# zhouzypaul/fql

Hardware: AMD Instinct MI355X
Metric: FQL gradient-steps/s (batch=256) (higher is better)
Workload: dtype f32

## Files before the change

fql_amd/csrc/fql_engine.hip:

```cpp
#include "../../include/fql_amd.h"
#include "fql_kernels.h"
#include "fql_conv.h"
#include "fql_chain.h"
#include "fql_aux.h"
#include "fql_ifql.h"
#include "fql_rebrac.h"
#include "fql_sac.h"
#include "fql_bc.h"
#include "fql_iql.h"
#include "fql_iqld.h"
#include "fql_cfgrl.h"
#include <hip/hip_ext.h>
#include "fql_aql.h"

#include <algorithm>
#include <cmath>
#include <cstdarg>
#include <cstdio>
#include <cstdlib>
#include <cstring>
#include <map>
#include <memory>
#include <random>
#include <string>
// ... 108 lines not shown
    size_t off = 0;
    ((off = ((off + alignof(T) - 1) & ~(alignof(T) - 1)) + sizeof(T)), ...);
    return off;
}
template <typename... Pm, typename... A>
Bound bind(void (*k)(Pm...), int grid, A&&... a) {
    static_assert(sizeof...(Pm) == sizeof...(A) && sizeof...(Pm) <= 2, "a bound launch takes the kernel's one or two arguments");
    static_assert(packed_bytes<Pm...>() <= FQL_BOUND_BYTES, "argument struct larger than Bound::args: raise FQL_BOUND_BYTES");
    Bound b;
    b.fn = (const void*)k;
    b.grid = (unsigned)grid;
    size_t off = 0;
    int n = 0;
    auto put = [&](auto v) {
        using T = decltype(v);
        off = (off + alignof(T) - 1) & ~(alignof(T) - 1);
        b.at[n++] = (int)off;
        std::memcpy(b.args + off, &v, sizeof(T));
        off += sizeof(T);
    };
    (put(static_cast<Pm>(a)), ...);
    b.len = (int)off;
    return b;
}

struct Op {
    OpType type;
    std::vector<const void*> reads, writes;
    GemmTask gemm;
    WgradTask wgrad;
    LnBwdTask ln;
    PrepArgs prep;
    PostOsArgs postos;
    LossCriticArgs lc;
    LossQArgs lq;
    LossBcArgs lb;
    LossActorArgs la;
    EulerFinishArgs ef;
    ConvArgs conv;
    PoolArgs pool;
    PoolBwdArgs poolb;
    ConvWgradArgs cw;
    ConvWredArgs cwr;
    EncDzArgs edz;
    ChainArgs chain;
    const ConvWprepTask* wprep_tasks = nullptr;
    int wprep_n = 0;
    int cw_grid = 0;
    int adam_c0 = 0, adam_n = -1;
    int adam_c1 = 0, adam_n1 = 0;
    int adam_polyak = -1;
    float adam_lr = 0.f;
    DevState* adam_st = nullptr;
    int fin_mode = 0;
    Bound k;
    int level = 0;
    int lane = 0;
    std::vector<int> deps;
};

struct Launch {
    OpType type;
    int grid = 0, ntasks = 0;
    size_t lds = 0;
    void* table = nullptr;
    Op op;
    bool pool_fused = false;
    int lane = 0;
    bool tmt2 = false, kbig = false, euler = false;
    double macs = 0.0;
    void *table_w = nullptr, *table_l = nullptr, *table_m = nullptr;
    int n_w = 0, n_l = 0, tile_w = 0, tile_l = 0, tile_m = 0;
    std::vector<GemmTask> dg_tasks;
    std::vector<GemmTask> h_gemm;
    std::vector<WgradTask> h_wgrad;
    std::vector<LnBwdTask> h_ln;
    std::vector<MiscTask> h_misc;
    std::shared_ptr<const SideArgs> ka_side;
    std::vector<int> waits;
    bool record_after = false;
    hipEvent_t ev = nullptr;
};

inline bool ka_tasks_env() {
    const char* e = getenv("FQL_KERNARG_TASKS");
    return !e || atoi(e) != 0;
}
inline std::shared_ptr<const SideArgs> ka_side_args(const Launch& L) {
    const size_t ng = L.h_gemm.size(), nw = L.h_wgrad.size(), nl = L.h_ln.size(), nm = L.h_misc.size();
    if (ng > FQL_KA_GEMM || nw > FQL_KA_WGRAD || nl > FQL_KA_LN || nm > FQL_KA_MISC) return nullptr;
    auto a = std::make_shared<SideArgs>();
    std::memset(a.get(), 0, sizeof(SideArgs));
    SideFront& f = a->f;
    f.tile_w = L.tile_w; f.tile_l = L.tile_l; f.tile_m = L.tile_m; f.tl = -1;
    for (int& v : f.g0) v = FQL_KA_FRONT_PAD;
    for (int& v : f.w0) v = FQL_KA_FRONT_PAD;
    for (int& v : f.l0) v = FQL_KA_FRONT_PAD;
    for (size_t i = 0; i < ng; ++i) { a->g[i] = L.h_gemm[i]; if (i) f.g0[i - 1] = L.h_gemm[i].tile0; }
    for (size_t i = 0; i < nw; ++i) { a->w[i] = L.h_wgrad[i]; if (i) f.w0[i - 1] = L.h_wgrad[i].tile0; }
    for (size_t i = 0; i < nl; ++i) { a->l[i] = L.h_ln[i]; if (i) f.l0[i - 1] = L.h_ln[i].tile0; }
    for (size_t i = 0; i < nm; ++i) a->m[i] = L.h_misc[i];
    return a;
}
struct Program {
    std::vector<Op> ops;
    std::vector<Launch> launches;
    bool lane_used[FQL_LANES] = {};
    hipEvent_t ev_fork = nullptr, ev_join[FQL_LANES] = {};
    hipGraph_t graph = nullptr;
    hipGraphExec_t exec = nullptr;
    int64_t macs = 0;
    AqlProgram aql;
    bool aql_tried = false;
};

template <typename P, typename IssueFn>
void issue_lanes(P& pr, hipStream_t s0, const hipStream_t* ls, bool fork, IssueFn&& issue) {
    auto lazy = [](hipEvent_t& e) { if (!e) HIP_CHECK(hipEventCreateWithFlags(&e, hipEventDisableTiming)); };
    bool side = false;
    if (ls) for (int l = 1; l < FQL_LANES; ++l) side |= pr.lane_used[l];
    if (side && fork) {
        lazy(pr.ev_fork);
        HIP_CHECK(hipEventRecord(pr.ev_fork, s0));
        for (int l = 1; l < FQL_LANES; ++l) if (pr.lane_used[l]) HIP_CHECK(hipStreamWaitEvent(ls[l], pr.ev_fork, 0));
    }
    for (auto& L : pr.launches) {
        const hipStream_t s = side && L.lane != 0 ? ls[L.lane] : s0;
        if (side)
            for (int w : L.waits) if (pr.launches[w].ev) HIP_CHECK(hipStreamWaitEvent(s, pr.launches[w].ev, 0));
        issue(L, s);
        if (side && L.record_after) {
            lazy(L.ev);
            HIP_CHECK(hipEventRecord(L.ev, s));
        }
    }
    if (side)
        for (int l = 1; l < FQL_LANES; ++l) {
            if (!pr.lane_used[l]) continue;
// ... 170 lines not shown
    int64_t* cf_rows = nullptr;
    uint32_t* cf_draws = nullptr;
    bool own_info() const { return kind == AgentKind::IQL || kind == AgentKind::IQLD; }
    uint64_t seed = 0;
    int device = 0;
    hipStream_t stream = nullptr;
    hipStream_t lane_streams[FQL_LANES] = {};
    bool allow64 = true;
    int emit_lane = 0;
    std::vector<Op>* defer_wgrads = nullptr;
    std::string err;

    Net nets[NUM_NETS];
    EncNet encs[NUM_ENC];
    ConvWprepTask* enc_wprep[NUM_ENC] = {nullptr, nullptr, nullptr, nullptr};
    int enc_nconv[NUM_ENC] = {0, 0, 0, 0};
    std::vector<void*> enc_allocs;
    bool visual = false;
    int enc_dim = 0;
    unsigned char* img_all = nullptr;
    EncBuf eb_c, eb_t, eb_bc, eb_os;
    size_t n_train = 0, n_total = 0, critic_size = 0;
    float *P = nullptr, *G = nullptr, *Mu = nullptr, *Nu = nullptr;
    std::vector<Leaf> leaves;
    int n_train_leaves = 0;
    AdamChunk* d_chunks = nullptr;
    float* d_partials = nullptr;
    int* d_leaf_range = nullptr;
    int n_chunks = 0;

    DevState* d_state = nullptr;
    SrcDesc* d_src = nullptr;
    SrcDesc h_src_shadow{};
    bool src_valid = false;
    SrcDesc* h_src_ring = nullptr;
    int src_ring_pos = 0;

    int B = 0;
    std::vector<void*> ws_allocs;
    float *in_obs = nullptr, *in_act = nullptr, *in_rew = nullptr, *in_mask = nullptr, *in_nobs = nullptr, *in_nact = nullptr;
    float* in_noise[5] = {nullptr, nullptr, nullptr, nullptr, nullptr};
    int64_t* in_idx = nullptr;
    float *X_os = nullptr, *X_bc = nullptr, *X_eu = nullptr, *X_c1 = nullptr, *X_c2 = nullptr, *X_ct = nullptr;
    float *vel = nullptr, *w_rew = nullptr, *w_mask = nullptr, *w_act = nullptr, *tgt = nullptr;
    float *X_e0 = nullptr, *C0 = nullptr, *Abuf[2] = {nullptr, nullptr}, *Vpart = nullptr;
    bool fused_euler = false;
    bool use_chain = false;
    int fill_lane_full = 1;
    std::vector<float*> wf_bc;
    float *wf_w0 = nullptr, *wf_w4 = nullptr;
    WfragTask* d_wfrag = nullptr;
    int wfrag_n = 0, wfrag_grid = 0;
    const bool ka_tasks = ka_tasks_env();
    std::vector<void*> chain_allocs;
    bool split_build = false;
    bool wide_tiles = false;
    bool split_ok = false;
    int vp_tiles = 0;
    int num_cus = 0;
    PassBuf p_os, p_os_bwd, p_bc, p_eu, p_c1[2], p_c2[2], p_ct[2];
    Program prog_fwdbwd, prog_opt, prog_loss;
    Program prog_opt_split;
    Program prog_full;
    int mod_chunk0[3] = {0, 0, 0}, mod_chunkn[3] = {0, 0, 0};
    Program prog_split;
    hipGraphExec_t split_exec[4] = {nullptr, nullptr, nullptr, nullptr};
    hipGraph_t split_graph[4] = {nullptr, nullptr, nullptr, nullptr};
    hipEvent_t ev_a = nullptr, ev_b = nullptr, ev_c = nullptr;
    bool split_begun = false;
    bool began = false;
    AqlRuntime aql;
    std::vector<AqlDispatch>* aql_rec = nullptr;
    bool last_update_aql = false;
    bool hip_dirty = true;
    void aql_drain() {
        if (!aql.up) return;
        try { aql.drain(); } catch (const AqlError& e) { throw HipError{e.msg}; }
    }

    float *ds_obs = nullptr, *ds_act = nullptr, *ds_rew = nullptr, *ds_mask = nullptr, *ds_nobs = nullptr;
    float* ds_row = nullptr;
    int64_t ds_size = 0, ds_cap = 0, ds_ptr = 0;
    unsigned char *ds_frames = nullptr, *ds_next_frames = nullptr;
    int64_t* ds_init = nullptr;
    int ds_fs = 0;
    float ds_paug = 0.f;
    float *rb_obs = nullptr, *rb_act = nullptr, *rb_rew = nullptr, *rb_mask = nullptr, *rb_nobs = nullptr;
    unsigned char *rb_frames = nullptr, *rb_next_frames = nullptr;
    int64_t* rb_init = nullptr;
    int64_t rb_size = 0, rb_cap = 0, rb_ptr = 0;
    int64_t* in_init = nullptr;
    int *in_crop = nullptr, *in_crop_user = nullptr;

    struct Eval {
        int n_pad = 0;
        std::vector<void*> allocs;
        float *X = nullptr, *Xf = nullptr, *tgt = nullptr;
        PassBuf p_os, p_eu;
        Program prog_os, prog_flow;
        float *st_obs = nullptr, *st_noise = nullptr, *st_out = nullptr;
        float* st_goal = nullptr;
        float *Xf2 = nullptr, *cfgs = nullptr;
        unsigned char* st_img = nullptr;
        EncBuf eb_os, eb_bc;
        Program prog_enc_os, prog_enc_bc;
        float* Xq = nullptr;
// ... 354 lines not shown
            lf.name = "modules_unc_embed/Embed_0/embedding";
            lf.ndim = 2;
            lf.shape[0] = 1; lf.shape[1] = gcfg.goal_dim; lf.shape[2] = lf.shape[3] = 1;
            lf.segs.push_back(Segment{emb_off, 1, gcfg.goal_dim, 1, pad16(gcfg.goal_dim)});
            lf.trainable = true;
            lf.train_id = tid++;
            leaves.push_back(lf);
        }
        n_train_leaves = tid;
        if (n_train_leaves > 256) invalid("too many trainable leaves (%d)", n_train_leaves);
        std::vector<AdamChunk> ch;
        for (const Leaf& lf : leaves) {
            if (!lf.trainable) continue;
            for (const Segment& s : lf.segs) {
                if (s.chunk_w > 0) {
                    for (int r = 0; r < s.rows_p; ++r) ch.push_back(AdamChunk{(int)(s.off + (size_t)r * s.cols_p), s.chunk_w, lf.train_id});
                    continue;
                }
                const size_t len = (size_t)s.rows_p * s.cols_p;
                for (size_t o = 0; o < len; o += 4096)
                    ch.push_back(AdamChunk{(int)(s.off + o), (int)std::min<size_t>(4096, len - o), lf.train_id});
            }
        }
        n_chunks = (int)ch.size();
        HIP_CHECK(hipMalloc((void**)&d_chunks, ch.size() * sizeof(AdamChunk)));
        HIP_CHECK(hipMemcpy(d_chunks, ch.data(), ch.size() * sizeof(AdamChunk), hipMemcpyHostToDevice));
        std::vector<int> range(n_train_leaves + 1, 0);
        for (const AdamChunk& c : ch) range[c.leaf + 1]++;
        for (int i = 0; i < n_train_leaves; ++i) range[i + 1] += range[i];
        {
            static const char* const trained[kNumKinds][3] = {
                {"modules_actor_bc_flow/", "modules_actor_onestep_flow/", "modules_critic/"},
                {"modules_actor_flow/", "modules_value/", "modules_critic/"},
                {"modules_actor/", "modules_critic/", "modules_critic/"},
                {"modules_actor/", "modules_alpha/", "modules_critic/"},
                {nullptr, nullptr, nullptr},
                {"modules_actor/", "modules_value/", "modules_critic/"},
                {"actor/", "value/", "critic/"},
                {nullptr, nullptr, nullptr}};
            const char* const* mods = trained[(int)kind];
            for (int m = 0; m < 3; ++m) {
                if (!mods[m]) { mod_chunk0[m] = 0; mod_chunkn[m] = n_chunks; continue; }
                int lo = 1 << 30, hi = -1;
                for (const Leaf& lf : leaves)
                    if (lf.trainable && lf.name.rfind(mods[m], 0) == 0) { lo = std::min(lo, lf.train_id); hi = std::max(hi, lf.train_id); }
                mod_chunk0[m] = range[lo];
                mod_chunkn[m] = range[hi + 1] - range[lo];
            }
        }
        HIP_CHECK(hipMalloc((void**)&d_leaf_range, range.size() * sizeof(int)));
        HIP_CHECK(hipMemcpy(d_leaf_range, range.data(), range.size() * sizeof(int), hipMemcpyHostToDevice));
        HIP_CHECK(hipMalloc((void**)&d_partials, (size_t)n_chunks * 4 * sizeof(float)));
        HIP_CHECK(hipMemset(d_partials, 0, (size_t)n_chunks * 4 * sizeof(float)));
    }

    const Leaf* find_leaf(const char* name) const {
        for (const Leaf& l : leaves)
            if (l.name == name) return &l;
        return nullptr;
    }
    static size_t leaf_count(const Leaf& l) {
        size_t n = 1;
        for (int i = 0; i < l.ndim; ++i) n *= (size_t)l.shape[i];
        return n;
    }
    void leaf_io(const Leaf& lf, float* arena, float* host, bool to_device) {
        HIP_CHECK(hipStreamSynchronize(stream));
        size_t ho = 0;
        for (const Segment& s : lf.segs) {
            HIP_CHECK(hipMemcpy2D(to_device ? (void*)(arena + s.off) : (void*)(host + ho), (to_device ? s.cols_p : s.cols) * sizeof(float),
                                  to_device ? (const void*)(host + ho) : (const void*)(arena + s.off),
                                  (to_device ? s.cols : s.cols_p) * sizeof(float), s.cols * sizeof(float), s.rows,
                                  to_device ? hipMemcpyHostToDevice : hipMemcpyDeviceToHost));
            ho += (size_t)s.rows * s.cols;
        }
    }

    void init_params() {
        std::vector<float> h(n_total, 0.f);
        std::mt19937_64 gen(seed * 0x9E3779B97F4A7C15ull + 0x1234567ull);
        for (int ni = 0; ni <= NET_OS; ++ni)
            for (const Layer& L : nets[ni].layers) {
                const bool actor_head = ni == NET_BC && &L == &nets[ni].layers.back();
                const double scale = !actor_head ? 1.0 : kind == AgentKind::REBRAC ? (double)rcfg.actor_fc_scale
                                     : kind == AgentKind::IQL ? 1e-2
                                                              : 1.0;
                if ((kind == AgentKind::BC || kind == AgentKind::IQLD) && actor_head) {
                    const double sd = std::sqrt(1.0 / (double)L.in) / 0.87962566103423978;
                    std::normal_distribution<double> Nd(0.0, 1.0);
                    for (int r = 0; r < L.in; ++r)
                        for (int c = 0; c < L.out; ++c) {
                            double v = Nd(gen);
                            while (v < -2.0 || v > 2.0) v = Nd(gen);
                            h[L.w + (size_t)r * L.out_p + c] = (float)(sd * v);
                        }
                    continue;
                }
                if (kind == AgentKind::SAC && actor_head) {
                    const int ad = cfg.act_dim, ap = pad16(ad);
                    const double lim = std::sqrt(6.0 * (double)scfg.actor_fc_scale / (double)(L.in + ad));
                    std::uniform_real_distribution<double> U(-lim, lim);
                    for (int c0 : {0, ap})
                        for (int r = 0; r < L.in; ++r)
                            for (int c = 0; c < ad; ++c) h[L.w + (size_t)r * L.out_p + c0 + c] = (float)U(gen);
                    continue;
                }
// ... 1118 lines not shown
            case OP_POOL_BWD: {
                const PoolBwdArgs& a = L.op.poolb;
                const size_t tot = (size_t)a.N * a.H * a.W * (a.C / 4);
                FQL_LAUNCH(fql_maxpool_bwd_kernel, dim3((unsigned)((tot + FQL_THREADS - 1) / FQL_THREADS)), dim3(FQL_THREADS), 0, s, a);
                break;
            }
            case OP_CONV_WGRAD:
                if (cfg.precision == 2) FQL_LAUNCH(fql_conv_wgrad_split_kernel, dim3(L.grid), dim3(FQL_THREADS), L.lds, s, (const ConvWgradArgs*)L.table, L.ntasks);
                else
                FQL_LAUNCH(fql_conv_wgrad_kernel, dim3(L.grid), dim3(FQL_THREADS), L.lds, s, (const ConvWgradArgs*)L.table, L.ntasks);
                break;
            case OP_CONV_WRED:
                FQL_LAUNCH(fql_conv_wgrad_reduce_kernel, dim3(L.grid), dim3(FQL_THREADS), 0, s, (const ConvWredArgs*)L.table, L.ntasks);
                break;
            case OP_ENC_DZ: {
                const EncDzArgs& a = L.op.edz;
                FQL_LAUNCH(fql_enc_dz_kernel, dim3((a.M * a.n + FQL_THREADS - 1) / FQL_THREADS), dim3(FQL_THREADS), 0, s, a);
                break;
            }
            case OP_CHAIN: {
                ChainArgs ca = L.op.chain; ca.tl = tl;
                ca.xg = chain_xg(ca.M, cfg.actor_hidden[0]);
                if (cfg.precision == 2 && ca.variant != 3) {
#define FQL_CHAIN_SPLIT(HH, VV) FQL_LAUNCH((fql_chain_split_kernel<HH, VV>), dim3((L.op.chain.M / 16) * (HH / 32)), dim3(FQL_CHAIN_THREADS), FQL_CHAIN_LDS_BYTES(HH), s, ca)
                    if (cfg.actor_hidden[0] == 512) { if (ca.variant == 0) FQL_CHAIN_SPLIT(512, 0); else if (ca.variant == 1) FQL_CHAIN_SPLIT(512, 1); else FQL_CHAIN_SPLIT(512, 2); }
                    else { if (ca.variant == 0) FQL_CHAIN_SPLIT(256, 0); else if (ca.variant == 1) FQL_CHAIN_SPLIT(256, 1); else FQL_CHAIN_SPLIT(256, 2); }
#undef FQL_CHAIN_SPLIT
                }
                else {
#define FQL_CHAIN_F32(HH, VV) FQL_LAUNCH((fql_chain_kernel<HH, VV>), dim3((L.op.chain.M / 16) * (HH / 32)), dim3(FQL_CHAIN_THREADS), FQL_CHAIN_LDS_BYTES(HH), s, ca)
                    if (cfg.actor_hidden[0] == 512) { if (ca.variant == 0) FQL_CHAIN_F32(512, 0); else if (ca.variant == 1) FQL_CHAIN_F32(512, 1); else if (ca.variant == 2) FQL_CHAIN_F32(512, 2); else FQL_CHAIN_F32(512, 3); }
                    else { if (ca.variant == 0) FQL_CHAIN_F32(256, 0); else if (ca.variant == 1) FQL_CHAIN_F32(256, 1); else if (ca.variant == 2) FQL_CHAIN_F32(256, 2); else FQL_CHAIN_F32(256, 3); }
#undef FQL_CHAIN_F32
                }
                break;
            }
            case OP_WFRAG:
                FQL_LAUNCH(fql_wfrag_kernel, dim3(wfrag_grid), dim3(FQL_THREADS), 0, s, (const WfragTask*)d_wfrag, wfrag_n, tl);
                break;
            case OP_DGRAD0: {
                Dgrad0Args a{};
                a.ntasks = (int)L.dg_tasks.size(); a.col0 = L.op.gemm.i1;
                for (int i = 0; i < a.ntasks; ++i) a.t[i] = L.dg_tasks[i];
                FQL_LAUNCH(fql_dgrad0_kernel, dim3(a.ntasks * (L.op.gemm.M / 16)), dim3(FQL_THREADS), 0, s, a);
                break;
            }
            case OP_HEAD_DGRAD:
                FQL_LAUNCH(fql_head_dgrad_kernel, dim3((L.op.gemm.M / 16) * (L.op.gemm.N / 64)), dim3(FQL_THREADS), 0, s, L.op.gemm);
                break;
            case OP_ADAM: {
                AdamArgs a{P, G, Mu, Nu, P + n_train, d_chunks, L.op.adam_st ? L.op.adam_st : d_state, d_partials, L.op.adam_c0,
                           L.op.adam_polyak >= 0 ? L.op.adam_polyak : (int)critic_size, L.op.adam_lr > 0.f ? L.op.adam_lr : cfg.lr, cfg.tau, tl,
                           L.op.adam_n1 > 0 ? L.op.adam_n : -1, L.op.adam_c1};
                FQL_LAUNCH(fql_adam_kernel, dim3(L.op.adam_n < 0 ? n_chunks : L.op.adam_n + L.op.adam_n1), dim3(FQL_THREADS), 0, s, a);
                break;
            }
            case OP_FINALIZE:
                FQL_LAUNCH(fql_finalize_kernel, dim3(1), dim3(FQL_THREADS), 0, s,
                                   FinalizeArgs{d_state, d_chunks, d_partials, d_leaf_range, n_chunks, n_train_leaves, L.op.fin_mode, tl});
                break;
            case OP_WGRAD: case OP_LNBWD: case OP_POSTOS: case OP_LOSS_CRITIC: case OP_LOSS_Q: case OP_LOSS_BC:
            case OP_PEC: case OP_XCHAIN: case OP_NUM_TYPES:
                throw HipError{"internal: op type " + std::to_string((int)L.type) + " has no launch of its own"};
            default: {
                const Bound& k = L.op.k;
                if (!k.fn) throw HipError{"internal: op type " + std::to_string((int)L.type) + " carries no bound launch"};
                alignas(16) unsigned char a[FQL_BOUND_BYTES];
                std::memcpy(a, k.args, (size_t)k.len);
                if (k.tl_at >= 0) std::memcpy(a + k.tl_at, &tl, sizeof tl);
                if (L.type == OP_IQLD_CFG) std::memcpy(a + offsetof(IqldCfgStepArgs, cfg), &sample_cfg, sizeof sample_cfg);
                void* argv[2] = {a + k.at[0], a + k.at[1]};
                if (aql_rec) aql_rec->push_back(AqlDispatch{k.fn, {k.grid, 1, 1}, {FQL_THREADS, 1, 1}, 0, std::vector<uint8_t>(a, a + k.len)});
                else if (prof_a) (void)hipExtLaunchKernel(k.fn, dim3(k.grid), dim3(FQL_THREADS), argv, 0, s, prof_a, prof_b, 0);
                else (void)hipLaunchKernel(k.fn, dim3(k.grid), dim3(FQL_THREADS), argv, 0, s);
                break;
            }
        }
    }

#undef FQL_LAUNCH
    void issue_of(const Program& pr, const Launch& L, hipStream_t s) {
        issue(L, s, &pr == &prog_full ? (int)(&L - pr.launches.data()) : -1);
    }
    void run_launches(Program& pr, hipStream_t s0, const hipStream_t* ls = nullptr, bool fork = true) {
        static const bool trace_l = getenv("FQL_TRACE") != nullptr;
        issue_lanes(pr, s0, ls, fork, [&](const Launch& L, hipStream_t s) {
            if (trace_l) {
                fprintf(stderr, "[fql] launch %d type %d lane %d grid %d waits %zu:", (int)(&L - pr.launches.data()), (int)L.type, L.lane, L.grid, L.waits.size());
                for (int w : L.waits) fprintf(stderr, " %d(lane %d)", w, pr.launches[w].lane);
                fprintf(stderr, "\n");
            }
            issue_of(pr, L, s);
        });
    }
    std::vector<AqlDispatch> record_dispatches(const Program& pr) {
        std::vector<AqlDispatch> rec;
        aql_rec = &rec;
        try {
            for (const Launch& L : pr.launches) issue_of(pr, L, nullptr);
        } catch (...) { aql_rec = nullptr; throw; }
        aql_rec = nullptr;
        if (rec.size() != pr.launches.size()) throw HipError{"internal: a launch did not record exactly one dispatch"};
        return rec;
    }

    void build_aql(Program& pr) {
// ... 394 lines not shown
                        if (m == 2) a.writes.push_back(P + n_train + c.w);
                    }
                const Layer& D = encs[ei].dense;
                a.reads.push_back(G + D.w); a.reads.push_back(G + D.b);
                a.writes.push_back(P + D.w);
                if (m == 2) a.writes.push_back(P + n_train + D.w);
            }
            for (int ni : net_ids)
                for (const Layer& L : nets[ni].layers) {
                    a.reads.push_back(G + L.w); a.reads.push_back(G + L.b);
                    a.writes.push_back(P + L.w);
                    if (L.ln) { a.reads.push_back(G + L.g); a.reads.push_back(G + L.be); a.writes.push_back(P + L.g); }
                    if (ni == NET_C0 || ni == NET_C1) a.writes.push_back(P + n_train + L.w);
                }
            emit_lane = lane;
            push(pr, a);
        }

    void build_opt_program(Program& pr, bool two_lanes) {
        DevState* st = d_state;
        if (two_lanes) {
            adam_for(pr, 2, {NET_C0, NET_C1}, 1);
            adam_for(pr, 0, {NET_BC}, 1);
            if (use_chain) { emit_lane = 1; emit_wfrag(pr); }
            adam_for(pr, 1, {NET_OS}, 0);
        } else {
            adam_for(pr, 2, {NET_C0, NET_C1, NET_BC, NET_OS}, 0, -2);
            if (use_chain) { emit_lane = 0; emit_wfrag(pr); }
        }
        Op f{};
        f.type = OP_FINALIZE;
        f.fin_mode = 1;
        f.reads = {d_partials + mod_chunk0[0] * 4, d_partials + mod_chunk0[1] * 4, d_partials + mod_chunk0[2] * 4, &st->info[0],
                   &st->info[4], &st->info[5], &st->info[7], &st->info[9]};
        f.writes = {&st->info[10], st};
        emit_lane = 0;
        push(pr, f);
    }
    void run_opt_split(hipStream_t s0, hipStream_t s1) {
        if (!ev_c) HIP_CHECK(hipEventCreateWithFlags(&ev_c, hipEventDisableTiming));
        if (!split_begun) HIP_CHECK(hipEventRecord(ev_c, s0));
        HIP_CHECK(hipStreamWaitEvent(s1, ev_c, 0));
        split_begun = false;
        const hipStream_t ls[FQL_LANES] = {s0, s1, s1, s1};
        run_launches(prog_opt_split, s0, ls, false);
    }

    void build_full_program(Program& pr) {
        build_step_program(pr, true);
        DevState* st = d_state;
        adam_for(pr, 2, {NET_C0, NET_C1, NET_BC}, fill_lane_full, 0);
        emit_wfrag(pr);
        adam_for(pr, 1, {NET_OS}, 0);
        Op f{};
        f.type = OP_FINALIZE;
        f.fin_mode = 1;
        f.reads = {d_partials + mod_chunk0[0] * 4, d_partials + mod_chunk0[1] * 4, d_partials + mod_chunk0[2] * 4, &st->info[0],
                   &st->info[4], &st->info[5], &st->info[7], &st->info[9]};
        f.writes = {&st->info[10], st};
        emit_lane = 0;
        push(pr, f);
    }

    FinalizeArgs fin_args(int do_grad_stats) const {
        return FinalizeArgs{d_state, d_chunks, d_partials, d_leaf_range, n_chunks, n_train_leaves, do_grad_stats, -1};
    }

    void build_ifql_program(Program& pr, bool with_grads) {
        const int od = cfg.obs_dim, ad = cfg.act_dim, ap = pad16(ad);
        DevState* st = d_state;
        const void *I_V = &st->info[IFQL_I_VALUE], *I_C = &st->info[IFQL_I_CRITIC], *I_A = &st->info[IFQL_I_ACTOR];
        wide_tiles = true;
        allow64 = true;
        emit_lane = 0;
        {
            Op op{};
            op.type = OP_IFQL_PREP;
            const IfqlPrepArgs iprep{d_src, st, seed, B, od, ad, nets[NET_OS].in_p(), nets[NET_C0].in_p(), nets[NET_BC].in_p(), ap,
                                     X_v, X_c1, X_bc, vel, w_rew, w_mask};
            op.k = bind(fql_ifql_prep_kernel, (iprep.B + 3) / 4, iprep);
            op.writes = {X_v, X_c1, X_bc, vel, w_rew, w_mask};
            push(pr, op);
        }
        emit_lane = 1;
        emit_forward(pr, p_v, with_grads);
        for (int e = 0; e < 2; ++e) emit_forward(pr, p_ct[e], false);
        {
            Op op{};
            op.type = OP_IFQL_LOSS_V;
            const IfqlValueArgs iv{p_v.out, p_ct[0].out, p_ct[1].out, with_grads ? p_v.dz.back() : nullptr, st, B, expectile};
            op.k = bind(fql_ifql_loss_value_kernel, 1, iv);
            op.reads = {p_v.out, p_ct[0].out, p_ct[1].out};
            op.writes = {I_V};
            if (with_grads) op.writes.push_back(p_v.dz.back());
            push(pr, op);
        }
        if (with_grads) emit_backward(pr, p_v, 0, B, true, false);
        emit_forward(pr, p_bc, with_grads);
        {
            Op op{};
            op.type = OP_LOSS_BC;
            op.lb = LossBcArgs{p_bc.out, vel, with_grads ? p_bc.dz.back() : nullptr, st, B, ad, ap, with_grads ? 1 : 0};
            op.reads = {p_bc.out, vel};
            op.writes = {I_A};
            if (with_grads) op.writes.push_back(p_bc.dz.back());
            push(pr, op);
// ... 2037 lines not shown
        HIP_CHECK(hipMemset(h->G, 0, h->n_train * sizeof(float)));
        HIP_CHECK(hipMemset(h->Mu, 0, h->n_train * sizeof(float)));
        HIP_CHECK(hipMemset(h->Nu, 0, h->n_train * sizeof(float)));
        h->build_enc_weights();
        h->build_leaves();
        h->init_params();
        h->build_chain_weights();
        h->refresh_chain_weights(h->stream);
        HIP_CHECK(hipMalloc((void**)&h->d_state, sizeof(DevState)));
        if (h->own_info()) {
            HIP_CHECK(hipMalloc((void**)&h->iql_info, 2 * IQL_INFO_STRIDE * sizeof(float)));
            HIP_CHECK(hipMemset(h->iql_info, 0, 2 * IQL_INFO_STRIDE * sizeof(float)));
        }
        HIP_CHECK(hipMalloc((void**)&h->d_src, sizeof(SrcDesc)));
        HIP_CHECK(hipHostMalloc((void**)&h->h_src_ring, 64 * sizeof(SrcDesc), hipHostMallocDefault));
        HIP_CHECK(hipHostMalloc((void**)&h->h_info_ring, fql_engine::kInfoRing * 32 * sizeof(float), hipHostMallocDefault));
        for (auto& e : h->info_ev) HIP_CHECK(hipEventCreateWithFlags(&e, hipEventDisableTiming));
        DevState st{};
        st.rng_step = 0; st.adam_count = 0; st.train_step = 1; st.b1pow = 1.0; st.b2pow = 1.0; st.grad_scale = 1.0f; st.lam = 1.0f;
        const float ninf = -INFINITY, pinf = INFINITY;
        int bi; std::memcpy(&bi, &ninf, 4); st.gmax = bi >= 0 ? bi : bi ^ 0x7FFFFFFF;
        std::memcpy(&bi, &pinf, 4); st.gmin = bi >= 0 ? bi : bi ^ 0x7FFFFFFF;
        HIP_CHECK(hipMemcpy(h->d_state, &st, sizeof st, hipMemcpyHostToDevice));
        if (kind == AgentKind::IQLD) {
            HIP_CHECK(hipMalloc((void**)&h->d_state_a, sizeof(DevState)));
            HIP_CHECK(hipMemcpy(h->d_state_a, &st, sizeof st, hipMemcpyHostToDevice));
        }
        if (kind == AgentKind::CFGRL) {
            HIP_CHECK(hipMalloc((void**)&h->d_gsrc, sizeof(CfgrlSrc)));
            HIP_CHECK(hipMemset(h->d_gsrc, 0, sizeof(CfgrlSrc)));
            HIP_CHECK(hipHostMalloc((void**)&h->h_gsrc_ring, 64 * sizeof(CfgrlSrc), hipHostMallocDefault));
        }
        h->build_workspace(cfg->batch_size);
    } catch (const Invalid& e) {
        g_create_error = e.msg; fql_destroy(h); return FQL_E_INVALID;
    } catch (const HipError& e) {
        g_create_error = e.msg; fql_destroy(h); return FQL_E_HIP;
    }
    *out = h;
    return FQL_OK;
}

int fql_destroy(fql_handle h) {
    if (!h) return FQL_OK;
    if (h->group) { h->err = "fql_destroy: the handle is a member of an agent group (fql_group_destroy first)"; return FQL_E_STATE; }
    try { h->aql_drain(); } catch (...) {}
    if (h->stream) hipStreamSynchronize(h->stream);
    hipDeviceSynchronize();
    h->free_workspace();
    h->aql.shutdown();
    for (auto* m : {&h->evals, &h->sweeps})
        for (auto& kv : *m)
            for (void* p : kv.second->allocs) hipFree(p);
    hipFree(h->P); hipFree(h->G); hipFree(h->Mu); hipFree(h->Nu); hipFree(h->d_chunks); hipFree(h->d_partials); hipFree(h->d_leaf_range); hipFree(h->d_state); hipFree(h->d_src); hipFree(h->d_emb); hipFree(h->iql_info); hipFree(h->d_state_a);
    if (h->h_src_ring) hipHostFree(h->h_src_ring);
    hipFree(h->d_gsrc); hipFree(h->ds_final); hipFree(h->ds_reps);
    if (h->h_gsrc_ring) hipHostFree(h->h_gsrc_ring);
    if (h->h_info_ring) hipHostFree(h->h_info_ring);
    for (auto& e : h->info_ev) if (e) hipEventDestroy(e);
    hipFree(h->ds_obs); hipFree(h->ds_act); hipFree(h->ds_rew); hipFree(h->ds_mask); hipFree(h->ds_nobs); hipFree(h->ds_row);
    hipFree(h->ds_frames); hipFree(h->ds_next_frames); hipFree(h->ds_init);
    hipFree(h->rb_obs); hipFree(h->rb_act); hipFree(h->rb_rew); hipFree(h->rb_mask); hipFree(h->rb_nobs);
    hipFree(h->rb_frames); hipFree(h->rb_next_frames); hipFree(h->rb_init);
    for (void* q : h->enc_allocs) hipFree(q);
    for (void* q : h->chain_allocs) hipFree(q);
    if (h->stream) hipStreamDestroy(h->stream);
    for (hipStream_t s : h->lane_streams) if (s) hipStreamDestroy(s);
    delete h;
    return FQL_OK;
}

int fql_set_batch_size(fql_handle h, int batch_size) {
    if (!h) return FQL_E_INVALID;
    if (h->group) { h->err = "fql_set_batch_size: the handle is a member of an agent group (fql_group_destroy first)"; return FQL_E_STATE; }
    FQL_TRY(h, { if (batch_size != h->B) h->build_workspace(batch_size); });
}

int fql_num_leaves(fql_handle h) { return h ? (int)h->leaves.size() : FQL_E_INVALID; }

int fql_leaf_info(fql_handle h, int index, char* name, int name_cap, int* ndim, int64_t shape[4]) {
    if (!h) return FQL_E_INVALID;
    FQL_TRY(h, {
        if (index < 0 || index >= (int)h->leaves.size()) invalid("leaf index %d out of range", index);
        const Leaf& l = h->leaves[index];
        if (name && name_cap > 0) { std::strncpy(name, l.name.c_str(), name_cap - 1); name[name_cap - 1] = 0; }
        if (ndim) *ndim = l.ndim;
        if (shape) for (int i = 0; i < 4; ++i) shape[i] = l.shape[i];
    });
}

static int leaf_rw(fql_handle h, const char* leaf, float* host, size_t n, int which, bool to_device) {
    if (!h) return FQL_E_INVALID;
    try {
        h->group_fence();
        h->hip_touch();
        if (!leaf || !host) invalid("leaf/host pointer must not be NULL");
        const Leaf* l = h->find_leaf(leaf);
        if (!l) { h->err = std::string("unknown leaf: ") + leaf; return FQL_E_NOTFOUND; }
        if (n != fql_engine::leaf_count(*l)) invalid("leaf %s has %zu elements, got %zu", leaf, fql_engine::leaf_count(*l), n);
        float* arena = h->P;
        if (which >= 0) {
            if (!l->trainable && which >= 0) {
                if (to_device) return FQL_OK;
                std::memset(host, 0, n * sizeof(float));
                return FQL_OK;
            }
            arena = which == 0 ? h->Mu : h->Nu;
// ... 1515 lines not shown
```

fql_amd/csrc/fql_kernels.h:

```cpp
#pragma once
#include <hip/hip_runtime.h>
#include <stdint.h>

typedef float f32x4 __attribute__((ext_vector_type(4)));

#define FQL_GAS __attribute__((address_space(1)))
__device__ __forceinline__ float ldg(const float* p) { return *(const FQL_GAS float*)p; }
__device__ __forceinline__ f32x4 ldg4(const float* p) { return *(const FQL_GAS f32x4*)p; }
__device__ __forceinline__ void stg(float* p, float v) { *(FQL_GAS float*)p = v; }
__device__ __forceinline__ void stg4(float* p, f32x4 v) { *(FQL_GAS f32x4*)p = v; }

#define FQL_THREADS 256

struct FastDiv {
    unsigned m;
    int d;
    __device__ __forceinline__ explicit FastDiv(int dd) : m(dd > 1 ? 0xFFFFFFFFu / (unsigned)dd + 1u : 0u), d(dd) {}
    __device__ __forceinline__ FastDiv(int dd, unsigned long long max_x) : m(dd > 1 && max_x * (unsigned long long)dd < (1ull << 32) ? 0xFFFFFFFFu / (unsigned)dd + 1u : 0u), d(dd) {}
    __device__ __forceinline__ int div(int x) const { return m ? (int)__umulhi((unsigned)x, m) : (d == 1 ? x : (int)((unsigned)x / (unsigned)d)); }
    __device__ __forceinline__ void divmod(int x, int& q, int& r) const { q = div(x); r = x - q * d; }
};

__device__ __forceinline__ float frcp(int d) { return __builtin_amdgcn_rcpf((float)d); }
__device__ __forceinline__ int sdiv(int x, float rd) { return (int)(((float)x + 0.5f) * rd); }
// ... 1895 lines not shown
    if (threadIdx.x == 0) P.st->info[5] = t / (float)n;
}

struct LossActorArgs {
    const float* a_raw;
    const float* tgt;
    const float *dxa, *dxb;
    float* da;
    DevState* st;
    int B, od, ad, inp_c, ap, want_grad;
    float alpha;
};
__device__ __forceinline__ void fql_loss_actor_body(const LossActorArgs& P, float* sh) {
    const int n = P.B * P.ad;
    const float gs = P.alpha * 2.0f / (float)n;
    float s = 0.f;
    for (int e = threadIdx.x; e < n; e += FQL_THREADS) {
        const int b = sdiv(e, frcp(P.ad)), a = e - b * P.ad;
        const float ar = P.a_raw[(size_t)b * P.ap + a];
        const float d = ar - P.tgt[(size_t)b * P.ap + a];
        s += d * d;
        if (P.want_grad) {
            float g = gs * d;
            if (ar > -1.0f && ar < 1.0f) {
                const size_t o = (size_t)b * P.inp_c + P.od + a;
                g += P.dxa[o] + P.dxb[o];
            }
            P.da[(size_t)b * P.ap + a] = g;
        }
    }
    const float t = block_sum(s, sh);
    if (threadIdx.x == 0) {
        const float distill = t / (float)n;
        P.st->info[6] = distill;
        P.st->info[4] = P.st->info[5] + P.alpha * distill + P.st->info[7];
    }
}

__global__ __launch_bounds__(FQL_THREADS) void fql_loss_actor_kernel(LossActorArgs P) { __shared__ float sh[4]; fql_loss_actor_body(P, sh); }
__global__ __launch_bounds__(FQL_THREADS) void fql_loss_actor_multi_kernel(const LossActorArgs* __restrict__ args) { __shared__ float sh[4]; const LossActorArgs P = args[blockIdx.y]; fql_loss_actor_body(P, sh); }

enum : int { MISC_POSTOS = 0, MISC_LOSS_CRITIC, MISC_LOSS_Q, MISC_LOSS_BC };
struct MiscTask {
    int kind;
    union {
        PostOsArgs po;
        LossCriticArgs lc;
        LossQArgs lq;
        LossBcArgs lb;
    };
};

struct AdamChunk { int off, len, leaf; };
struct AdamArgs {
    float *P, *G, *Mu, *Nu, *T;
    const AdamChunk* chunks;
    DevState* st;
    float* partials;
    int chunk0;
    int critic_size;
    float lr, tau;
    int tl;
    int n0, chunk1;
};
__device__ __forceinline__ int f2ord(float f) {
    const int i = __float_as_int(f);
    return i >= 0 ? i : i ^ 0x7FFFFFFF;
}
__device__ __forceinline__ float ord2f(int i) { return __int_as_float(i >= 0 ? i : i ^ 0x7FFFFFFF); }

__device__ __forceinline__ void fql_adam_body(const AdamArgs& A) {
    __shared__ float sh[4];
    tl_enter(A.tl);
    const int cidx = (A.n0 < 0 || (int)blockIdx.x < A.n0) ? (int)blockIdx.x + A.chunk0 : (int)blockIdx.x - A.n0 + A.chunk1;
    const AdamChunk ch = A.chunks[cidx];
    const float c1 = (float)(1.0 - A.st->b1pow * 0.9), c2 = (float)(1.0 - A.st->b2pow * 0.999);
    const float gsc = A.st->grad_scale;
    float ss = 0.f, mx = -INFINITY, mn = INFINITY;
    const int n4 = ch.len >> 2;
#pragma unroll
    for (int it = 0; it < 4; ++it) {
        const int i = threadIdx.x + it * FQL_THREADS;
        if (i < n4) {
            const int o = ch.off + 4 * i;
            f32x4 g = ldg4(A.G + o);
            const f32x4 p = ldg4(A.P + o);
            f32x4 m = ldg4(A.Mu + o);
            f32x4 v = ldg4(A.Nu + o);
            f32x4 pn;
#pragma unroll
            for (int e = 0; e < 4; ++e) {
                const float ge = g[e] * gsc;
                m[e] = 0.9f * m[e] + 0.1f * ge;
                v[e] = 0.999f * v[e] + 0.001f * ge * ge;
                const float mh = m[e] / c1, vh = v[e] / c2;
                pn[e] = p[e] - A.lr * (mh / (sqrtf(vh) + 1e-8f));
                ss += ge * ge; mx = fmaxf(mx, ge); mn = fminf(mn, ge);
            }
            stg4(A.Mu + o, m);
            stg4(A.Nu + o, v);
            stg4(A.P + o, pn);
            if (o < A.critic_size) {
                f32x4 t = ldg4(A.T + o);
#pragma unroll
                for (int e = 0; e < 4; ++e) t[e] = p[e] * A.tau + t[e] * (1.0f - A.tau);
                stg4(A.T + o, t);
            }
        }
    }
    const float tss = block_sum(ss, sh);
    const float tmx = block_max(mx, sh), tmn = -block_max(-mn, sh);
    if (threadIdx.x == 0) {
        float* pp = A.partials + 4 * (size_t)cidx;
        pp[0] = tss; pp[1] = tmx; pp[2] = tmn;
    }
    tl_exit(A.tl);
}
__global__ __launch_bounds__(FQL_THREADS) void fql_adam_kernel(AdamArgs A) { fql_adam_body(A); }
__global__ __launch_bounds__(FQL_THREADS) void fql_adam_multi_kernel(const AdamArgs* __restrict__ args) { const AdamArgs A = ((const FQL_CONST_AS AdamArgs*)args)[blockIdx.y]; fql_adam_body(A); }

struct FinalizeArgs {
    DevState* st;
    const AdamChunk* chunks;
    const float* partials;
    const int* leaf_range;
    int n_chunks, nleaves, do_grad_stats;
    int tl;
};
__device__ __forceinline__ void fql_finalize_body(const FinalizeArgs& A) {
    __shared__ float sh[4];
    __shared__ float leafn[256];
    DevState* st = A.st;
    tl_enter(A.tl);
    if (!A.do_grad_stats) return;
    float mx = -INFINITY, mn = INFINITY;
    for (int cidx = threadIdx.x; cidx < A.n_chunks; cidx += FQL_THREADS) {
        mx = fmaxf(mx, A.partials[4 * cidx + 1]);
        mn = fminf(mn, A.partials[4 * cidx + 2]);
    }
    for (int base = 0; base < A.nleaves; base += 64) {
        const int l = base + (threadIdx.x >> 2), sub = threadIdx.x & 3;
        float s = 0.f;
        if (l < A.nleaves) {
            const int b = A.leaf_range[l], e = A.leaf_range[l + 1];
            const int per = (e - b + 3) >> 2;
            const int lo = b + sub * per, hi = min(e, lo + per);
            for (int cidx = lo; cidx < hi; ++cidx) s += A.partials[4 * cidx];
        }
        s += __shfl_xor(s, 1);
        s += __shfl_xor(s, 2);
        if (l < A.nleaves && sub == 0) leafn[l] = sqrtf(s);
    }
    const float tmx = block_max(mx, sh), tmn = -block_max(-mn, sh);
    __syncthreads();
    if (threadIdx.x == 0) {
        float nrm = 0.f;
        for (int i = 0; i < A.nleaves; ++i) nrm += leafn[i];
        st->info[10] = fmaxf(tmx, 0.0f);
        st->info[11] = fminf(tmn, 0.0f);
        st->info[12] = nrm;
        st->rng_step += 1;
        st->adam_count += 1;
        st->train_step += 1;
        st->b1pow *= 0.9;
        st->b2pow *= 0.999;
    }
}
__global__ __launch_bounds__(FQL_THREADS) void fql_finalize_kernel(FinalizeArgs A) { fql_finalize_body(A); }
__global__ __launch_bounds__(FQL_THREADS) void fql_finalize_multi_kernel(const FinalizeArgs* __restrict__ args) { const FinalizeArgs A = args[blockIdx.y]; fql_finalize_body(A); }

struct EulerFinishArgs {
    const float* a_in;
    const float* evp;
    const float* eb;
    float* tgt;
    int M, ad, ap, ntp, a_ld;
    float scale;
};
__device__ __forceinline__ void fql_euler_finish_body(const EulerFinishArgs& P) {
    const int e = blockIdx.x * FQL_THREADS + threadIdx.x;
    if (e >= P.M * P.ad) return;
    const int r = sdiv(e, frcp(P.ad)), j = e - r * P.ad;
    float pv[32];
#pragma unroll
    for (int tp = 0; tp < 32; ++tp) pv[tp] = ldg(P.evp + ((size_t)min(tp, P.ntp - 1) * P.M + r) * P.ap + j);
    float sum = 0.f;
#pragma unroll
    for (int tp = 0; tp < 32; ++tp) sum += (tp < P.ntp) ? pv[tp] : 0.f;
    stg(P.tgt + (size_t)r * P.ap + j, clip1(ldg(P.a_in + (size_t)r * P.a_ld + j) + (sum + ldg(P.eb + j)) * P.scale));
}
__global__ __launch_bounds__(FQL_THREADS) void fql_euler_finish_kernel(EulerFinishArgs P) { fql_euler_finish_body(P); }
__global__ __launch_bounds__(FQL_THREADS) void fql_euler_finish_multi_kernel(const EulerFinishArgs* __restrict__ args) { const EulerFinishArgs P = args[blockIdx.y]; fql_euler_finish_body(P); }

struct EncDzArgs {
    const float *dxa, *dxb;
    const float* z;
    float* dz;
    int M, n, ld;
};
__global__ __launch_bounds__(FQL_THREADS) void fql_enc_dz_kernel(const EncDzArgs P) {
    const int e = blockIdx.x * FQL_THREADS + threadIdx.x;
    if (e >= P.M * P.n) return;
    const int r = e / P.n, j = e - r * P.n;
    float g = ldg(P.dxa + (size_t)r * P.ld + j);
    if (P.dxb) g += ldg(P.dxb + (size_t)r * P.ld + j);
    stg(P.dz + e, g * ldg(P.z + e));
}

struct AssembleArgs {
    const float *obs, *noise;
    float* X;
    uint64_t key, seed;
    int n, n_pad, od, ad, inp;
};
__global__ __launch_bounds__(FQL_THREADS) void fql_assemble_kernel(AssembleArgs P) {
    const int wave = threadIdx.x >> 6, lane = threadIdx.x & 63;
    const int b = blockIdx.x * 4 + wave;
    if (b >= P.n_pad) return;
    for (int j = lane; j < P.inp; j += 64) {
// ... 145 lines not shown
```

Baseline: 2919.

## Fuse Adam finalize into last Adam block via atomic ticket

Each Adam block writes its partials, then takes a ticket with an agent-scope atomic. The block that takes the last ticket runs the finalize reduction itself, which removes the separate finalize kernel launch and its dependency edge in the optimizer program. Finalize partial loads are also unrolled into batches of 4 and 8. This adds cross-block ordering that depends on atomics and relaxed loads, and is gated by an env var that defaults on.

Measured after the change: 2960 (median of 6 runs). 1.4% higher.

```diff
diff --git a/fql_amd/csrc/fql_engine.hip b/fql_amd/csrc/fql_engine.hip
--- a/fql_amd/csrc/fql_engine.hip
+++ b/fql_amd/csrc/fql_engine.hip
@@ -184,6 +184,7 @@
     int adam_polyak = -1;
     float adam_lr = 0.f;
     DevState* adam_st = nullptr;
+    bool adam_fin = false;
     int fin_mode = 0;
     Bound k;
     int level = 0;
@@ -216,6 +217,10 @@
 
 inline bool ka_tasks_env() {
     const char* e = getenv("FQL_KERNARG_TASKS");
+    return !e || atoi(e) != 0;
+}
+inline bool fused_tail_env() {
+    const char* e = getenv("FQL_FUSED_TAIL");
     return !e || atoi(e) != 0;
 }
 inline std::shared_ptr<const SideArgs> ka_side_args(const Launch& L) {
@@ -492,6 +497,8 @@
     WfragTask* d_wfrag = nullptr;
     int wfrag_n = 0, wfrag_grid = 0;
     const bool ka_tasks = ka_tasks_env();
+    const bool fused_tail = fused_tail_env();
+    unsigned* d_ticket = nullptr;
     std::vector<void*> chain_allocs;
     bool split_build = false;
     bool wide_tiles = false;
@@ -952,6 +959,8 @@
         HIP_CHECK(hipMemcpy(d_leaf_range, range.data(), range.size() * sizeof(int), hipMemcpyHostToDevice));
         HIP_CHECK(hipMalloc((void**)&d_partials, (size_t)n_chunks * 4 * sizeof(float)));
         HIP_CHECK(hipMemset(d_partials, 0, (size_t)n_chunks * 4 * sizeof(float)));
+        HIP_CHECK(hipMalloc((void**)&d_ticket, 16));
+        HIP_CHECK(hipMemset(d_ticket, 0, 16));
     }
 
     const Leaf* find_leaf(const char* name) const {
@@ -2176,6 +2185,11 @@
                 AdamArgs a{P, G, Mu, Nu, P + n_train, d_chunks, L.op.adam_st ? L.op.adam_st : d_state, d_partials, L.op.adam_c0,
                            L.op.adam_polyak >= 0 ? L.op.adam_polyak : (int)critic_size, L.op.adam_lr > 0.f ? L.op.adam_lr : cfg.lr, cfg.tau, tl,
                            L.op.adam_n1 > 0 ? L.op.adam_n : -1, L.op.adam_c1};
+                if (L.op.adam_fin) {
+                    a.ticket = d_ticket;
+                    a.ticket_n = n_chunks;
+                    a.fin = FinalizeArgs{d_state, d_chunks, d_partials, d_leaf_range, n_chunks, n_train_leaves, L.op.fin_mode, -1};
+                }
                 FQL_LAUNCH(fql_adam_kernel, dim3(L.op.adam_n < 0 ? n_chunks : L.op.adam_n + L.op.adam_n1), dim3(FQL_THREADS), 0, s, a);
                 break;
             }
@@ -2676,6 +2690,10 @@
         adam_for(pr, 2, {NET_C0, NET_C1, NET_BC}, fill_lane_full, 0);
         emit_wfrag(pr);
         adam_for(pr, 1, {NET_OS}, 0);
+        if (fused_tail && mod_chunkn[0] + mod_chunkn[1] + mod_chunkn[2] == n_chunks) {
+            for (Op& o : pr.ops) if (o.type == OP_ADAM) { o.adam_fin = true; o.fin_mode = 1; }
+            return;
+        }
         Op f{};
         f.type = OP_FINALIZE;
         f.fin_mode = 1;
@@ -4819,7 +4837,7 @@
     for (auto* m : {&h->evals, &h->sweeps})
         for (auto& kv : *m)
             for (void* p : kv.second->allocs) hipFree(p);
-    hipFree(h->P); hipFree(h->G); hipFree(h->Mu); hipFree(h->Nu); hipFree(h->d_chunks); hipFree(h->d_partials); hipFree(h->d_leaf_range); hipFree(h->d_state); hipFree(h->d_src); hipFree(h->d_emb); hipFree(h->iql_info); hipFree(h->d_state_a);
+    hipFree(h->P); hipFree(h->G); hipFree(h->Mu); hipFree(h->Nu); hipFree(h->d_chunks); hipFree(h->d_partials); hipFree(h->d_ticket); hipFree(h->d_leaf_range); hipFree(h->d_state); hipFree(h->d_src); hipFree(h->d_emb); hipFree(h->iql_info); hipFree(h->d_state_a);
     if (h->h_src_ring) hipHostFree(h->h_src_ring);
     hipFree(h->d_gsrc); hipFree(h->ds_final); hipFree(h->ds_reps);
     if (h->h_gsrc_ring) hipHostFree(h->h_gsrc_ring);
diff --git a/fql_amd/csrc/fql_kernels.h b/fql_amd/csrc/fql_kernels.h
--- a/fql_amd/csrc/fql_kernels.h
+++ b/fql_amd/csrc/fql_kernels.h
@@ -1971,6 +1971,14 @@
 };
 
 struct AdamChunk { int off, len, leaf; };
+struct FinalizeArgs {
+    DevState* st;
+    const AdamChunk* chunks;
+    const float* partials;
+    const int* leaf_range;
+    int n_chunks, nleaves, do_grad_stats;
+    int tl;
+};
 struct AdamArgs {
     float *P, *G, *Mu, *Nu, *T;
     const AdamChunk* chunks;
@@ -1981,6 +1989,9 @@
     float lr, tau;
     int tl;
     int n0, chunk1;
+    unsigned* ticket;
+    int ticket_n;
+    FinalizeArgs fin;
 };
 __device__ __forceinline__ int f2ord(float f) {
     const int i = __float_as_int(f);
@@ -1988,74 +1999,26 @@
 }
 __device__ __forceinline__ float ord2f(int i) { return __int_as_float(i >= 0 ? i : i ^ 0x7FFFFFFF); }
 
-__device__ __forceinline__ void fql_adam_body(const AdamArgs& A) {
-    __shared__ float sh[4];
-    tl_enter(A.tl);
-    const int cidx = (A.n0 < 0 || (int)blockIdx.x < A.n0) ? (int)blockIdx.x + A.chunk0 : (int)blockIdx.x - A.n0 + A.chunk1;
-    const AdamChunk ch = A.chunks[cidx];
-    const float c1 = (float)(1.0 - A.st->b1pow * 0.9), c2 = (float)(1.0 - A.st->b2pow * 0.999);
-    const float gsc = A.st->grad_scale;
-    float ss = 0.f, mx = -INFINITY, mn = INFINITY;
-    const int n4 = ch.len >> 2;
-#pragma unroll
-    for (int it = 0; it < 4; ++it) {
-        const int i = threadIdx.x + it * FQL_THREADS;
-        if (i < n4) {
-            const int o = ch.off + 4 * i;
-            f32x4 g = ldg4(A.G + o);
-            const f32x4 p = ldg4(A.P + o);
-            f32x4 m = ldg4(A.Mu + o);
-            f32x4 v = ldg4(A.Nu + o);
-            f32x4 pn;
-#pragma unroll
-            for (int e = 0; e < 4; ++e) {
-                const float ge = g[e] * gsc;
-                m[e] = 0.9f * m[e] + 0.1f * ge;
-                v[e] = 0.999f * v[e] + 0.001f * ge * ge;
-                const float mh = m[e] / c1, vh = v[e] / c2;
-                pn[e] = p[e] - A.lr * (mh / (sqrtf(vh) + 1e-8f));
-                ss += ge * ge; mx = fmaxf(mx, ge); mn = fminf(mn, ge);
-            }
-            stg4(A.Mu + o, m);
-            stg4(A.Nu + o, v);
-            stg4(A.P + o, pn);
-            if (o < A.critic_size) {
-                f32x4 t = ldg4(A.T + o);
-#pragma unroll
-                for (int e = 0; e < 4; ++e) t[e] = p[e] * A.tau + t[e] * (1.0f - A.tau);
-                stg4(A.T + o, t);
-            }
-        }
-    }
-    const float tss = block_sum(ss, sh);
-    const float tmx = block_max(mx, sh), tmn = -block_max(-mn, sh);
-    if (threadIdx.x == 0) {
-        float* pp = A.partials + 4 * (size_t)cidx;
-        pp[0] = tss; pp[1] = tmx; pp[2] = tmn;
-    }
-    tl_exit(A.tl);
-}
-__global__ __launch_bounds__(FQL_THREADS) void fql_adam_kernel(AdamArgs A) { fql_adam_body(A); }
-__global__ __launch_bounds__(FQL_THREADS) void fql_adam_multi_kernel(const AdamArgs* __restrict__ args) { const AdamArgs A = ((const FQL_CONST_AS AdamArgs*)args)[blockIdx.y]; fql_adam_body(A); }
-
-struct FinalizeArgs {
-    DevState* st;
-    const AdamChunk* chunks;
-    const float* partials;
-    const int* leaf_range;
-    int n_chunks, nleaves, do_grad_stats;
-    int tl;
-};
-__device__ __forceinline__ void fql_finalize_body(const FinalizeArgs& A) {
-    __shared__ float sh[4];
-    __shared__ float leafn[256];
+template <bool SC1>
+__device__ __forceinline__ float ld_partial(const float* p) {
+    if constexpr (SC1) return __hip_atomic_load((FQL_GAS float*)p, __ATOMIC_RELAXED, __HIP_MEMORY_SCOPE_AGENT);
+    else return *p;
+}
+template <bool SC1>
+__device__ __forceinline__ void fql_finalize_core(const FinalizeArgs& A, float* sh, float* leafn) {
     DevState* st = A.st;
-    tl_enter(A.tl);
     if (!A.do_grad_stats) return;
     float mx = -INFINITY, mn = INFINITY;
-    for (int cidx = threadIdx.x; cidx < A.n_chunks; cidx += FQL_THREADS) {
-        mx = fmaxf(mx, A.partials[4 * cidx + 1]);
-        mn = fminf(mn, A.partials[4 * cidx + 2]);
+    for (int c0 = threadIdx.x; c0 < A.n_chunks; c0 += 4 * FQL_THREADS) {
+        float vx[4], vn[4];
+#pragma unroll
+        for (int j = 0; j < 4; ++j) {
+            const int cidx = c0 + j * FQL_THREADS;
+            vx[j] = cidx < A.n_chunks ? ld_partial<SC1>(A.partials + 4 * cidx + 1) : -INFINITY;
+            vn[j] = cidx < A.n_chunks ? ld_partial<SC1>(A.partials + 4 * cidx + 2) : INFINITY;
+        }
+#pragma unroll
+        for (int j = 0; j < 4; ++j) { mx = fmaxf(mx, vx[j]); mn = fminf(mn, vn[j]); }
     }
     for (int base = 0; base < A.nleaves; base += 64) {
         const int l = base + (threadIdx.x >> 2), sub = threadIdx.x & 3;
@@ -2064,7 +2027,13 @@
             const int b = A.leaf_range[l], e = A.leaf_range[l + 1];
             const int per = (e - b + 3) >> 2;
             const int lo = b + sub * per, hi = min(e, lo + per);
-            for (int cidx = lo; cidx < hi; ++cidx) s += A.partials[4 * cidx];
+            for (int c0 = lo; c0 < hi; c0 += 8) {
+                float v[8];
+#pragma unroll
+                for (int j = 0; j < 8; ++j) v[j] = c0 + j < hi ? ld_partial<SC1>(A.partials + 4 * (c0 + j)) : 0.f;
+#pragma unroll
+                for (int j = 0; j < 8; ++j) if (c0 + j < hi) s += v[j];
+            }
         }
         s += __shfl_xor(s, 1);
         s += __shfl_xor(s, 2);
@@ -2084,6 +2053,79 @@
         st->b1pow *= 0.9;
         st->b2pow *= 0.999;
     }
+}
+
+__device__ __forceinline__ void fql_adam_body(const AdamArgs& A) {
+    __shared__ float sh[4];
+    __shared__ float leafn[256];
+    tl_enter(A.tl);
+    const int cidx = (A.n0 < 0 || (int)blockIdx.x < A.n0) ? (int)blockIdx.x + A.chunk0 : (int)blockIdx.x - A.n0 + A.chunk1;
+    const AdamChunk ch = A.chunks[cidx];
+    const float c1 = (float)(1.0 - A.st->b1pow * 0.9), c2 = (float)(1.0 - A.st->b2pow * 0.999);
+    const float gsc = A.st->grad_scale;
+    float ss = 0.f, mx = -INFINITY, mn = INFINITY;
+    const int n4 = ch.len >> 2;
+#pragma unroll
+    for (int it = 0; it < 4; ++it) {
+        const int i = threadIdx.x + it * FQL_THREADS;
+        if (i < n4) {
+            const int o = ch.off + 4 * i;
+            f32x4 g = ldg4(A.G + o);
+            const f32x4 p = ldg4(A.P + o);
+            f32x4 m = ldg4(A.Mu + o);
+            f32x4 v = ldg4(A.Nu + o);
+            f32x4 pn;
+#pragma unroll
+            for (int e = 0; e < 4; ++e) {
+                const float ge = g[e] * gsc;
+                m[e] = 0.9f * m[e] + 0.1f * ge;
+                v[e] = 0.999f * v[e] + 0.001f * ge * ge;
+                const float mh = m[e] / c1, vh = v[e] / c2;
+                pn[e] = p[e] - A.lr * (mh / (sqrtf(vh) + 1e-8f));
+                ss += ge * ge; mx = fmaxf(mx, ge); mn = fminf(mn, ge);
+            }
+            stg4(A.Mu + o, m);
+            stg4(A.Nu + o, v);
+            stg4(A.P + o, pn);
+            if (o < A.critic_size) {
+                f32x4 t = ldg4(A.T + o);
+#pragma unroll
+                for (int e = 0; e < 4; ++e) t[e] = p[e] * A.tau + t[e] * (1.0f - A.tau);
+                stg4(A.T + o, t);
+            }
+        }
+    }
+    const float tss = block_sum(ss, sh);
+    const float tmx = block_max(mx, sh), tmn = -block_max(-mn, sh);
+    float* pp = A.partials + 4 * (size_t)cidx;
+    if (!A.ticket) {
+        if (threadIdx.x == 0) { pp[0] = tss; pp[1] = tmx; pp[2] = tmn; }
+        tl_exit(A.tl);
+        return;
+    }
+    if (threadIdx.x == 0) {
+        const u32x4 v = {__float_as_uint(tss), __float_as_uint(tmx), __float_as_uint(tmn), 0u};
+        __builtin_amdgcn_raw_buffer_store_b128(v, __builtin_amdgcn_make_buffer_rsrc(pp, 0, 16, 0x00020000), 0, 0, 16);
+        asm volatile("s_waitcnt vmcnt(0)" ::: "memory");
+        const unsigned t = __hip_atomic_fetch_add((FQL_GAS unsigned*)A.ticket, 1u, __ATOMIC_RELAXED, __HIP_MEMORY_SCOPE_AGENT);
+        sh[0] = t == (unsigned)(A.ticket_n - 1) ? 1.0f : 0.0f;
+    }
+    __syncthreads();
+    const bool last = sh[0] != 0.0f;
+    if (last) {
+        fql_finalize_core<true>(A.fin, sh, leafn);
+        if (threadIdx.x == 0) __hip_atomic_store((FQL_GAS unsigned*)A.ticket, 0u, __ATOMIC_RELAXED, __HIP_MEMORY_SCOPE_AGENT);
+    }
+    tl_exit(A.tl);
+}
+__global__ __launch_bounds__(FQL_THREADS) void fql_adam_kernel(AdamArgs A) { fql_adam_body(A); }
+__global__ __launch_bounds__(FQL_THREADS) void fql_adam_multi_kernel(const AdamArgs* __restrict__ args) { const AdamArgs A = ((const FQL_CONST_AS AdamArgs*)args)[blockIdx.y]; fql_adam_body(A); }
+
+__device__ __forceinline__ void fql_finalize_body(const FinalizeArgs& A) {
+    __shared__ float sh[4];
+    __shared__ float leafn[256];
+    tl_enter(A.tl);
+    fql_finalize_core<false>(A, sh, leafn);
 }
 __global__ __launch_bounds__(FQL_THREADS) void fql_finalize_kernel(FinalizeArgs A) { fql_finalize_body(A); }
 __global__ __launch_bounds__(FQL_THREADS) void fql_finalize_multi_kernel(const FinalizeArgs* __restrict__ args) { const FinalizeArgs A = args[blockIdx.y]; fql_finalize_body(A); }
```
